# eduard-permyakov/permafrost-engine

Measured on AMD Instinct MI355X. Metric: agent-steps/sec (+ flow-field cells/sec), every chunk field rebuilt + every agent stepped per tick, higher is better.
Workload: dtype u64-bitmask/u8 fields, f32 agents (f64 exp); 1 GPU; BASELINE configs[2]: 1024x1024 cells, 64 flow fields = 16384 chunk fields, 100000 agents; map_chunks=16, flow_fields=64, agents=100000, hz=20, dynamic_obstacles=0, parallelism=requests by destination + uid slabs x1, 1 all-gather (16 B/agent) per tick, ranks=1, rccl_ranks=1, backend=none, tile_exchange=auto, requests=reference planner fixture, has_dest_los=device lookup, initial_velocities=flow aligned, fields_ahead=True, tick_driver=c (navhip_tick_run), library=libnavhip.so (in-tree)

## Files before the change

### permafrost-engine_amd/csrc/field_kernels.hip

```cpp
#include "navhip_internal.h"

#include "wave_bits.h"

__device__ __forceinline__ bool req_uses_bfs(const nh_map_view &map, const navhip_field_req &rq,
                                             int force_generic)
{
    if(force_generic) return false;
    if(rq.type == NAVHIP_TARGET_NEAREST_PATHABLE || (rq.flags & NAVHIP_REQ_ISLAND_NEAREST)) return false;
    const nh_layer_view &L = map.layers[rq.layer];
    return L.unit_cost[(int)rq.chunk_r * map.w + rq.chunk_c] != 0;
}

__device__ __forceinline__ uint16_t portal_first_iid(const uint16_t *li, int r0, int c0, int r1, int c1)
{
    for(int r = r0; r <= r1; r++)
        for(int c = c0; c <= c1; c++) {
            const uint16_t v = li[r * 64 + c];
            if(v != NAVHIP_ISLAND_NONE) return v;
        }
    return NAVHIP_ISLAND_NONE;
}

__device__ __forceinline__ bool req_prepare(const nh_map_view &map, navhip_field_req &rq)
{
    const nh_layer_view &L = map.layers[rq.layer];
    const bool portal = rq.type == NAVHIP_TARGET_PORTAL;
    if((rq.flags & NAVHIP_REQ_IF_CHANGED) && L.changed) {
        bool ch = L.changed[(int)rq.chunk_r * map.w + rq.chunk_c] != 0;
        if(portal) ch |= L.changed[(int)rq.next_chunk_r * map.w + rq.next_chunk_c] != 0;
        if(!ch) return false;
    }
    if((rq.flags & NAVHIP_REQ_LIVE_IIDS) && portal && L.local_islands) {
        rq.port_iid = portal_first_iid(L.local_islands + ((size_t)((int)rq.chunk_r * map.w + rq.chunk_c) << 12),
                                       rq.port_r0, rq.port_c0, rq.port_r1, rq.port_c1);
        rq.next_iid = portal_first_iid(L.local_islands + ((size_t)((int)rq.next_chunk_r * map.w + rq.next_chunk_c) << 12),
                                       rq.next_r0, rq.next_c0, rq.next_r1, rq.next_c1);
        if(rq.port_iid == NAVHIP_ISLAND_NONE || rq.next_iid == NAVHIP_ISLAND_NONE) return false;
    }
    return true;
}

__device__ __forceinline__ bool next_tile_matches(const nh_map_view &map, const navhip_field_req &rq,
                                                  int gr, int gc)
{
    if(gr < 0 || gc < 0) return false;
    int cr2 = gr >> 6, cc2 = gc >> 6, r2 = gr & 63, c2 = gc & 63;
    if(cr2 != rq.next_chunk_r || cc2 != rq.next_chunk_c) return false;
    if(cr2 >= map.h || cc2 >= map.w) return false;
    if(r2 < rq.next_r0 || r2 > rq.next_r1 || c2 < rq.next_c0 || c2 > rq.next_c1) return false;
    const uint16_t *li = map.layers[rq.layer].local_islands;
    return li[((size_t)(cr2 * map.w + cc2) << 12) + r2 * 64 + c2] == rq.next_iid;
}

__device__ __forceinline__ bool portal_seed(const nh_map_view &map, const navhip_field_req &rq,
                                            int r, int c, bool passable)
{
    if(!passable) return false;
    if(r < rq.port_r0 || r > rq.port_r1 || c < rq.port_c0 || c > rq.port_c1) return false;
    const uint16_t *li = map.layers[rq.layer].local_islands;
    size_t cbase = (size_t)((int)rq.chunk_r * map.w + rq.chunk_c) << 12;
    if(rq.port_iid != NAVHIP_ISLAND_NONE && li[cbase + r * 64 + c] != rq.port_iid) return false;
    int gr = rq.chunk_r * 64 + r, gc = rq.chunk_c * 64 + c;
    return next_tile_matches(map, rq, gr - 1, gc) || next_tile_matches(map, rq, gr + 1, gc)
        || next_tile_matches(map, rq, gr, gc - 1) || next_tile_matches(map, rq, gr, gc + 1);
}

__device__ __forceinline__ uint32_t portal_fix_dir(const navhip_field_req &rq)
{
    if(rq.next_chunk_r < rq.chunk_r) return NAVHIP_FD_N;
    if(rq.next_chunk_r > rq.chunk_r) return NAVHIP_FD_S;
    if(rq.next_chunk_c < rq.chunk_c) return NAVHIP_FD_W;
    return NAVHIP_FD_E;
}

__global__ __launch_bounds__(256) void k_derive(const uint8_t *cost, const uint16_t *blockers,
                                                uint64_t *passmask, uint64_t *probemask, uint8_t *unit_cost,
                                                const uint8_t *factions, uint64_t *facmask, uint16_t *facany,
                                                const uint32_t *chunk_list, int n)
{
    int wave = (blockIdx.x * 256 + threadIdx.x) >> 6;
    int lane = threadIdx.x & 63;
    if(wave >= n) return;
    uint32_t chunk = chunk_list ? chunk_list[wave] : (uint32_t)wave;
    const uint8_t  *cb = cost + ((size_t)chunk << 12);
    const uint16_t *bl = blockers ? blockers + ((size_t)chunk << 12) : nullptr;
    uint64_t mine = 0, path = 0, blocked = 0;
    bool nonunit = false;
    for(int r = 0; r < 64; r++) {
        uint32_t cst = cb[r * 64 + lane];
        uint32_t blk = bl ? bl[r * 64 + lane] : 0;
        uint64_t m = __ballot(cst != NAVHIP_COST_IMPASSABLE && blk == 0);
        uint64_t mp = __ballot(cst != NAVHIP_COST_IMPASSABLE), mb = __ballot(blk > 0);
        nonunit |= (cst != NAVHIP_COST_IMPASSABLE && cst != 1);
        if(lane == r) { mine = m; path = mp; blocked = mb; }
    }
    passmask[(size_t)chunk * 64 + lane] = mine;
    probemask[((size_t)chunk * 64 + lane) * 2]     = path;
    probemask[((size_t)chunk * 64 + lane) * 2 + 1] = blocked;
    bool any_nonunit = __any(nonunit);
    if(lane == 0) unit_cost[chunk] = any_nonunit ? 0 : 1;
    if(factions) {
        const uint8_t *fa = factions + ((size_t)chunk * NAVHIP_MAX_FACTIONS << 12) + lane * 64;
        uint32_t any = 0;
        for(int f = 0; f < NAVHIP_MAX_FACTIONS; f++) {
            const uint64_t m = nz_row_mask(fa + ((size_t)f << 12));
            facmask[((size_t)chunk * NAVHIP_MAX_FACTIONS + f) * 64 + lane] = m;
            if(__ballot(m != 0)) any |= 1u << f;
        }
        if(lane == 0) facany[chunk] = (uint16_t)any;
    }
}

void nh_launch_derive(navhip_ctx *ctx, int layer, const uint32_t *d_chunk_list, int n, hipStream_t s)
{
    navhip_layer &L = ctx->layers[layer];
    int blocks = (n + 3) / 4;
    hipLaunchKernelGGL(k_derive, dim3(blocks), dim3(256), 0, s, L.cost, L.blockers, L.passmask, L.probemask,
                       L.unit_cost, L.factions, L.facmask, L.facany, d_chunk_list, n);
}

__device__ __forceinline__ uint64_t faction_pass_row(const nh_layer_view &L, int chunk, int lane, uint32_t enemies)
{
    const uint64_t *pm = L.probemask + ((size_t)chunk * 64 + lane) * 2;
    const uint64_t path = pm[0], blocked = pm[1];
    if(!L.facmask) return path;
    uint64_t friends = 0;
    uint32_t fs = __builtin_amdgcn_readfirstlane((int)(L.facany[chunk] & ~enemies & ((1u << NAVHIP_MAX_FACTIONS) - 1u)));
    const uint64_t *fm = L.facmask + (size_t)chunk * NAVHIP_MAX_FACTIONS * 64 + lane;
    while(fs) {
        const int f = __builtin_ctz(fs);
        fs &= fs - 1;
        friends |= fm[f * 64];
    }
    return path & ~(blocked & friends);
}

#define NH_MAXP 12
#define BFS_WAVES 4

template <bool WANT_INTEG>
__global__ __launch_bounds__(BFS_WAVES * 64) void k_field_bfs(nh_map_view map, const navhip_field_req *reqs,
                                                   int n, uint8_t *dirs, float *integ,
                                                   int force_generic, int32_t *gen_list, int gen_slot,
                                                   const int32_t *out_slot)
{
    __shared__ __attribute__((aligned(16))) uint8_t stage[BFS_WAVES][NH_CELLS];

    const int wib  = threadIdx.x >> 6;
    const int wave = blockIdx.x * BFS_WAVES + wib;
    const int lane = threadIdx.x & 63;
    if(wave >= n) return;

    navhip_field_req rq = reqs[wave];
    if(!req_uses_bfs(map, rq, force_generic)) {
        if(lane == 0) gen_list[2 + atomicAdd(&gen_list[gen_slot], 1)] = wave;
        return;
    }
    if(!req_prepare(map, rq)) return;

    const nh_layer_view &L = map.layers[rq.layer];
    const int chunk = (int)rq.chunk_r * map.w + rq.chunk_c;
    const u64x pass = mk(rq.faction_id == NAVHIP_FACTION_ID_NONE ? L.passmask[(size_t)chunk * 64 + lane]
                                                                 : faction_pass_row(L, chunk, lane, rq.enemies));

    u64x seeds = u64x{0, 0};
    if(rq.type == NAVHIP_TARGET_TILE) {
        if(lane == rq.tile_r) seeds = mk(1ull << rq.tile_c) & pass;
    }else{
        if(rq.port_c0 == rq.port_c1) {
            bool s = portal_seed(map, rq, lane, rq.port_c0, (to64(pass) >> rq.port_c0) & 1);
            if(s) seeds = mk(1ull << rq.port_c0);
        }else{
            for(int r = rq.port_r0; r <= rq.port_r1; r++) {
                uint64_t prow = __shfl(to64(pass), r);
                bool s = portal_seed(map, rq, r, lane, (prow >> lane) & 1);
                uint64_t m = __ballot(s);
                if(lane == r) seeds = mk(m);
            }
        }
    }

    u64x open = andn(pass, seeds);
    u64x frontier = seeds;
    u64x pl[NH_MAXP];
#pragma unroll
    for(int k = 0; k < NH_MAXP; k++) pl[k] = u64x{0, 0};

    int level = 0;
#define NH_BFS_LEVEL(NLOW)                                                                   \
    {                                                                                        \
        u64x nw = bfs_reach(frontier, open);                                                 \
        if(!__any(nz(nw))) break;                                                            \
        level++;                                                                             \
        pl[0] = pl[0] ^ open;                                                                \
        if(NLOW > 1) pl[1] = pl[1] ^ open;                                                   \
        if(NLOW > 2) pl[2] = pl[2] ^ open;                                                   \
        if(NLOW > 3) {                                                                       \
            const int tz = __builtin_ctz(level);          \
            _Pragma("unroll")                                                                \
            for(int k = 3; k < NH_MAXP; k++) {                                               \
                if(k <= tz) pl[k] = pl[k] ^ open;                                            \
            }                                                                                \
        }                                                                                    \
        open = andn(open, nw);                                                               \
        frontier = nw;                                                                       \
    }
    for(;;) {
        NH_BFS_LEVEL(1) NH_BFS_LEVEL(2) NH_BFS_LEVEL(1) NH_BFS_LEVEL(3)
        NH_BFS_LEVEL(1) NH_BFS_LEVEL(2) NH_BFS_LEVEL(1) NH_BFS_LEVEL(4)
    }
#undef NH_BFS_LEVEL
    const u64x reach = andn(pass, open);
#pragma unroll
    for(int k = 0; k < NH_MAXP; k++) pl[k] = pl[k] & reach;

    const int P = 32 - __builtin_clz((unsigned)level + 1);

    if(WANT_INTEG) {
        float *out = integ + ((size_t)wave << 12);
        for(int c = 0; c < 64; c++) {
            uint32_t d = 0;
#pragma unroll
            for(int k = 0; k < NH_MAXP; k++) d |= (uint32_t)((to64(pl[k]) >> c) & 1) << k;
            bool fin = (to64(reach) >> c) & 1;
            out[lane * 64 + c] = fin ? (float)d : __builtin_inff();
        }
    }

    u64x anybit = u64x{0, 0};
#pragma unroll
    for(int k = 0; k < NH_MAXP; k++) anybit = anybit | pl[k];
    const u64x zero = andn(reach, anybit);
    const u64x act  = reach & anybit;

    const u64x rN = from_n(reach), rS = from_s(reach), rW = from_w(reach), rE = from_e(reach);
    u64x eqN, eqS, eqW, eqE;
    {
        const u64x m0 = pl[0], m1 = pl[1];
        u64x n0, n1;
        n0 = from_n(pl[0]); n1 = from_n(pl[1]); eqN = andn(n0 ^ m0, n1 ^ n0 ^ m1) & rN;
        n0 = from_s(pl[0]); n1 = from_s(pl[1]); eqS = andn(n0 ^ m0, n1 ^ n0 ^ m1) & rS;
        n0 = from_w(pl[0]); n1 = from_w(pl[1]); eqW = andn(n0 ^ m0, n1 ^ n0 ^ m1) & rW;
        n0 = from_e(pl[0]); n1 = from_e(pl[1]); eqE = andn(n0 ^ m0, n1 ^ n0 ^ m1) & rE;
    }

    u64x neNW = u64x{0, 0}, neNE = neNW, neSW = neNW, neSE = neNW;
    {
        u64x b1 = u64x{~0u, ~0u};
        u64x b2 = u64x{~0u, ~0u};
#pragma unroll
        for(int k = 0; k < NH_MAXP; k++) {
            if(k < P) {
                u64x e = pl[k] ^ b1;  b1 = andn(b1, pl[k]);
                u64x f = e ^ b2;      b2 = andn(b2, e);
                u64x up = from_n(pl[k]), dn = from_s(pl[k]);
                neNW = neNW | (from_w(up) ^ f);
                neNE = neNE | (from_e(up) ^ f);
                neSW = neSW | (from_w(dn) ^ f);
                neSE = neSE | (from_e(dn) ^ f);
            }
        }
    }
    const u64x eqNW = andn(from_w(rN), neNW), eqNE = andn(from_e(rN), neNE);
    const u64x eqSW = andn(from_w(rS), neSW), eqSE = andn(from_e(rS), neSE);

    const u64x hasD = (eqNW & rN & rW) | (eqNE & rN & rE) | (eqSW & rS & rW) | (eqSE & rS & rE);
    const u64x h = act & hasD;
    const u64x g = andn(act, hasD);

    const u64x mN  = g & eqN;
    const u64x mS  = andn(g & eqS, eqN);
    const u64x mE  = andn(g & eqE, eqN | eqS);
    const u64x mW  = andn(g & eqW, eqN | eqS | eqE);
    const u64x mNW = h & eqNW;
    const u64x mNE = andn(h & eqNE, eqNW);
    const u64x mSW = andn(h & eqSW, eqNW | eqNE);
    const u64x mSE = andn(h & eqSE, eqNW | eqNE | eqSW);

    u64x D0 = mNW | mNE | mE | mS;
    u64x D1 = mN | mNE | mSW | mS;
    u64x D2 = mW | mE | mSW | mS;
    u64x D3 = mSE;
    if(rq.type == NAVHIP_TARGET_PORTAL) {
        uint32_t fd = portal_fix_dir(rq);
        if(fd & 1) D0 = D0 | zero;
        if(fd & 2) D1 = D1 | zero;
        if(fd & 4) D2 = D2 | zero;
    }

    uint8_t *out = dirs + ((size_t)(out_slot ? out_slot[wave] : wave) << 12);
    uint8_t *st = stage[wib];
    const bool inout = (rq.flags & NAVHIP_REQ_INOUT) != 0;
    if(inout) {
#pragma unroll
        for(int j = 0; j < 4; j++)
            *(uint4*)(st + j * 1024 + lane * 16) = *(const uint4*)(out + j * 1024 + lane * 16);
    }
    __builtin_amdgcn_wave_barrier();
    {
        uint32_t *row = (uint32_t*)(st + lane * 64);
        const uint64_t d0 = to64(D0), d1 = to64(D1), d2 = to64(D2), d3 = to64(D3);
        const uint64_t rc = to64(reach);
#pragma unroll
        for(int j = 0; j < 16; j++) {
            uint32_t b0 = (((uint32_t)(d0 >> (4 * j)) & 0xf) * 0x00204081u) & 0x01010101u;
            uint32_t b1 = (((uint32_t)(d1 >> (4 * j)) & 0xf) * 0x00204081u) & 0x01010101u;
            uint32_t b2 = (((uint32_t)(d2 >> (4 * j)) & 0xf) * 0x00204081u) & 0x01010101u;
            uint32_t b3 = (((uint32_t)(d3 >> (4 * j)) & 0xf) * 0x00204081u) & 0x01010101u;
            uint32_t v = b0 | (b1 << 1) | (b2 << 2) | (b3 << 3);
            if(inout) {
                uint32_t rm = ((((uint32_t)(rc >> (4 * j)) & 0xf) * 0x00204081u) & 0x01010101u) * 0xffu;
                v = (v & rm) | (row[j] & ~rm);
            }
            row[j] = v;
        }
    }
    __builtin_amdgcn_wave_barrier();
#pragma unroll
    for(int j = 0; j < 4; j++)
        *(uint4*)(out + j * 1024 + lane * 16) = *(const uint4*)(st + j * 1024 + lane * 16);
}

struct generic_lds {
    uint32_t dist[NH_CELLS];
    __attribute__((aligned(16))) uint8_t pc[NH_CELLS];
    uint8_t raw[NH_CELLS];
    uint8_t fl[NH_CELLS];
    int s_list[128], s_dmin[128], s_nlist, s_D;
};

__device__ void field_generic_one(generic_lds &S, const nh_map_view &map, const navhip_field_req *reqs,
                                  int ri, uint8_t *dirs, float *integ, int force_generic,
                                  const int32_t *out_slot)
{
    uint32_t (&dist)[NH_CELLS] = S.dist;
    uint8_t (&pc)[NH_CELLS] = S.pc;
    uint8_t (&raw)[NH_CELLS] = S.raw;
    uint8_t (&fl)[NH_CELLS] = S.fl;
    int (&s_list)[128] = S.s_list;
    int (&s_dmin)[128] = S.s_dmin;
    int &s_nlist = S.s_nlist, &s_D = S.s_D;

    const int t = threadIdx.x;
    navhip_field_req rq = reqs[ri];
    if(req_uses_bfs(map, rq, force_generic)) return;
    if(!req_prepare(map, rq)) return;

    const nh_layer_view &L = map.layers[rq.layer];
    const size_t cbase = (size_t)((int)rq.chunk_r * map.w + rq.chunk_c) << 12;
    const bool faction = rq.faction_id != NAVHIP_FACTION_ID_NONE;
    const bool modeA = rq.type == NAVHIP_TARGET_NEAREST_PATHABLE;
    const bool modeB = !modeA && (rq.flags & NAVHIP_REQ_ISLAND_NEAREST) != 0;

#pragma unroll 4
    for(int k = 0; k < 16; k++) {
        int i = k * 256 + t;
        uint32_t cst = L.cost[cbase + i];
        uint32_t blk = L.blockers ? L.blockers[cbase + i] : 0;
        bool passable;
        if(cst == NAVHIP_COST_IMPASSABLE) {
            passable = false;
        }else if(!faction) {
            passable = (blk == 0);
        }else{
            bool enemies_only = true;
            if(L.factions) {
                const uint8_t *fp = L.factions + cbase * NAVHIP_MAX_FACTIONS + i;
                for(int f = 0; f < NAVHIP_MAX_FACTIONS; f++) {
                    if(fp[(size_t)f << 12] && !(rq.enemies & (1u << f))) { enemies_only = false; break; }
                }
            }
            passable = enemies_only || (blk == 0);
        }
        pc[i] = passable ? (uint8_t)cst : (uint8_t)NAVHIP_COST_IMPASSABLE;
        raw[i] = (uint8_t)cst;
        fl[i] = (cst != NAVHIP_COST_IMPASSABLE && blk == 0) ? 1 : 0;
        dist[i] = NH_INF_U32;
    }
    if(t == 0) { s_nlist = 0; s_D = 0x7fffffff; }
    if(t < 128) s_dmin[t] = 0x7fffffff;
    __syncthreads();

    if(modeA) {
        const int start = rq.tile_r * 64 + rq.tile_c;
        if(t == 0) fl[start] |= 2;
        __syncthreads();
        if(!(fl[start] & 1)) {
            for(;;) {
                int changed = 0;
#pragma unroll 4
                for(int k = 0; k < 16; k++) {
                    int i = k * 256 + t;
                    if(fl[i] & 3) continue;
                    int r = i >> 6, c = i & 63;
                    bool nb = (r > 0 && (fl[i - 64] & 2)) || (r < 63 && (fl[i + 64] & 2))
                           || (c > 0 && (fl[i - 1] & 2)) || (c < 63 && (fl[i + 1] & 2));
                    if(nb) { fl[i] |= 2; changed = 1; }
                }
                if(!__syncthreads_or(changed)) break;
            }
#pragma unroll 4
            for(int k = 0; k < 16; k++) {
                int i = k * 256 + t;
                if(!(fl[i] & 1)) continue;
                int r = i >> 6, c = i & 63;
                bool nb = (r > 0 && (fl[i - 64] & 2)) || (r < 63 && (fl[i + 64] & 2))
                       || (c > 0 && (fl[i - 1] & 2)) || (c < 63 && (fl[i + 1] & 2));
                if(nb) dist[i] = 0;
            }
        }else if(t == 0) {
            dist[start] = 0;
        }
        __syncthreads();
        for(;;) {
            int changed = 0;
#pragma unroll 4
            for(int k = 0; k < 16; k++) {
                int i = k * 256 + t;
                if(fl[i] & 1) continue;
                int r = i >> 6, c = i & 63;
                uint32_t m = NH_INF_U32;
                if(r > 0)  m = min(m, dist[i - 64]);
                if(r < 63) m = min(m, dist[i + 64]);
                if(c > 0)  m = min(m, dist[i - 1]);
                if(c < 63) m = min(m, dist[i + 1]);
                if(m < NH_INF_U32) {
                    uint32_t nd = m + raw[i];
                    if(nd < dist[i]) { dist[i] = nd; changed = 1; }
                }
            }
            if(!__syncthreads_or(changed)) break;
        }
    }else{
        if(rq.type == NAVHIP_TARGET_TILE) {
            if(t == 0) {
                int i = rq.tile_r * 64 + rq.tile_c;
                if(pc[i] != NAVHIP_COST_IMPASSABLE) {
                    if(modeB) s_list[s_nlist++] = i; else dist[i] = 0;
                }
            }
        }else{
            int nr = rq.port_r1 - rq.port_r0 + 1, nc = rq.port_c1 - rq.port_c0 + 1;
            for(int j = t; j < nr * nc; j += 256) {
                int r = rq.port_r0 + j / nc, c = rq.port_c0 + j % nc;
                if(portal_seed(map, rq, r, c, pc[r * 64 + c] != NAVHIP_COST_IMPASSABLE)) {
                    if(modeB) { int p = atomicAdd(&s_nlist, 1); if(p < 128) s_list[p] = r * 64 + c; }
                    else dist[r * 64 + c] = 0;
                }
            }
        }
        __syncthreads();
        if(modeB) {
            if(t == 0 && s_nlist == 0 && rq.type == NAVHIP_TARGET_TILE)
                s_list[s_nlist++] = rq.tile_r * 64 + rq.tile_c;
            __syncthreads();
            const int nl = min(s_nlist, 128);
            const uint16_t *li = L.local_islands + cbase;
            const uint16_t *gi = L.islands ? L.islands + cbase : nullptr;
            const uint32_t want = rq.aux_iid;
            for(int q = 0; q < nl; q++) {
                const int f = s_list[q], fr = f >> 6, fc = f & 63;
                const uint32_t giid = gi ? gi[f] : NAVHIP_ISLAND_NONE;
                int best = 0x7fffffff;
#pragma unroll 4
                for(int k = 0; k < 16; k++) {
                    int i = k * 256 + t;
                    if(!(fl[i] & 1)) continue;
                    if(want != NAVHIP_ISLAND_NONE && li[i] != want) continue;
                    if(giid != NAVHIP_ISLAND_NONE && gi[i] != giid) continue;
                    int d = abs((i >> 6) - fr) + abs((i & 63) - fc);
                    best = min(best, d);
                }
                if(best < 0x7fffffff) atomicMin(&s_dmin[q], best);
            }
            __syncthreads();
            if(t == 0) {
                int D = 0x7fffffff;
                for(int q = 0; q < nl; q++) D = min(D, s_dmin[q]);
                s_D = D;
            }
            __syncthreads();
            const int D = s_D;
            if(D < 0x7fffffff) {
                for(int q = 0; q < nl; q++) {
                    if(s_dmin[q] != D) continue;
                    const int f = s_list[q], fr = f >> 6, fc = f & 63;
                    const uint32_t giid = gi ? gi[f] : NAVHIP_ISLAND_NONE;
#pragma unroll 4
                    for(int k = 0; k < 16; k++) {
                        int i = k * 256 + t;
                        if(!(fl[i] & 1)) continue;
                        if(want != NAVHIP_ISLAND_NONE && li[i] != want) continue;
                        if(giid != NAVHIP_ISLAND_NONE && gi[i] != giid) continue;
                        if(abs((i >> 6) - fr) + abs((i & 63) - fc) == D) dist[i] = 0;
                    }
                }
            }
            __syncthreads();
        }

        for(;;) {
            int changed = 0;
#pragma unroll 4
            for(int k = 0; k < 16; k++) {
                int i = k * 256 + t;
                uint32_t cst = pc[i];
                if(cst == NAVHIP_COST_IMPASSABLE) continue;
                int r = i >> 6, c = i & 63;
                uint32_t m = NH_INF_U32;
                if(r > 0)  m = min(m, dist[i - 64]);
                if(r < 63) m = min(m, dist[i + 64]);
                if(c > 0)  m = min(m, dist[i - 1]);
                if(c < 63) m = min(m, dist[i + 1]);
                if(m < NH_INF_U32) {
                    uint32_t nd = m + cst;
                    if(nd < dist[i]) { dist[i] = nd; changed = 1; }
                }
            }
            if(!__syncthreads_or(changed)) break;
        }
    }

    const bool inout = (rq.flags & NAVHIP_REQ_INOUT) != 0 || modeA || modeB;
    uint8_t *out = dirs + ((size_t)(out_slot ? out_slot[ri] : ri) << 12);
    const uint32_t fixdir = (rq.type == NAVHIP_TARGET_PORTAL) ? portal_fix_dir(rq) : NAVHIP_FD_NONE;
    uint8_t res[16];
#pragma unroll 4
    for(int k = 0; k < 16; k++) {
        int i = k * 256 + t;
        int r = i >> 6, c = i & 63;
        uint32_t d = dist[i];
        uint32_t dir;
        if(d >= NH_INF_U32) {
            dir = inout ? out[i] : NAVHIP_FD_NONE;
        }else if(d == 0) {
            dir = modeA ? out[i] : fixdir;
        }else{
            const uint32_t I = NH_INF_U32;
            uint32_t dn = r > 0  ? dist[i - 64] : I, ds = r < 63 ? dist[i + 64] : I;
            uint32_t dw = c > 0  ? dist[i - 1]  : I, de = c < 63 ? dist[i + 1]  : I;
            uint32_t dnw = (r > 0  && c > 0)  ? dist[i - 65] : I;
            uint32_t dne = (r > 0  && c < 63) ? dist[i - 63] : I;
            uint32_t dsw = (r < 63 && c > 0)  ? dist[i + 63] : I;
            uint32_t dse = (r < 63 && c < 63) ? dist[i + 65] : I;
            uint32_t mc = min(min(dn, ds), min(dw, de));
            if(dn < I && dw < I) mc = min(mc, dnw);
            if(dn < I && de < I) mc = min(mc, dne);
            if(ds < I && dw < I) mc = min(mc, dsw);
            if(ds < I && de < I) mc = min(mc, dse);
            if(dn == mc)       dir = NAVHIP_FD_N;
            else if(ds == mc)  dir = NAVHIP_FD_S;
            else if(de == mc)  dir = NAVHIP_FD_E;
            else if(dw == mc)  dir = NAVHIP_FD_W;
            else if(dnw == mc) dir = NAVHIP_FD_NW;
            else if(dne == mc) dir = NAVHIP_FD_NE;
            else if(dsw == mc) dir = NAVHIP_FD_SW;
            else               dir = NAVHIP_FD_SE;
        }
        res[k] = (uint8_t)dir;
        if(integ) integ[((size_t)ri << 12) + i] = (d >= NH_INF_U32) ? __builtin_inff() : (float)d;
    }
    __syncthreads();
#pragma unroll
    for(int k = 0; k < 16; k++) pc[k * 256 + t] = res[k];
    __syncthreads();
    *(uint4*)(out + t * 16) = *(const uint4*)(pc + t * 16);
}

__global__ __launch_bounds__(256) void k_field_generic(nh_map_view map, const navhip_field_req *reqs,
                                                       int n, uint8_t *dirs, float *integ,
                                                       int force_generic, int32_t *gen_list, int gen_slot,
                                                       const int32_t *out_slot)
{
    __shared__ generic_lds S;
    const int count = gen_list ? gen_list[gen_slot] : n;
    if(gen_list && blockIdx.x == 0 && threadIdx.x == 0) gen_list[gen_slot ^ 1] = 0;
    for(int w = blockIdx.x; w < count; w += gridDim.x) {
        const int ri = gen_list ? gen_list[2 + w] : w;
        field_generic_one(S, map, reqs, ri, dirs, integ, force_generic, out_slot);
        __syncthreads();
    }
}

int nh_launch_fields(navhip_ctx *ctx, const navhip_field_req *d_reqs, int n, uint8_t *d_dirs,
                     float *d_integ, int32_t *d_gen_list, hipStream_t s, const int32_t *d_out_slot)
{
    nh_map_view mv;
    nh_fill_map_view(ctx, &mv);
    const int force_generic = ctx->field_kernel_mode == 1;
    const int gen_slot = force_generic ? 0 : (int)(ctx->gen_launches++ & 1);
    if(!force_generic) {
        dim3 grid((n + BFS_WAVES - 1) / BFS_WAVES);
        if(d_integ)
            hipLaunchKernelGGL(k_field_bfs<true>, grid, dim3(BFS_WAVES * 64), 0, s, mv, d_reqs, n, d_dirs,
                               d_integ, force_generic, d_gen_list, gen_slot, d_out_slot);
        else
            hipLaunchKernelGGL(k_field_bfs<false>, grid, dim3(BFS_WAVES * 64), 0, s, mv, d_reqs, n, d_dirs,
                               d_integ, force_generic, d_gen_list, gen_slot, d_out_slot);
    }
    bool heavy = force_generic;
    for(int l = 0; l < NAVHIP_NAV_LAYER_MAX; l++) heavy = heavy || (ctx->layers[l].cost && ctx->layers[l].nonunit_costs);
    const int gmax = heavy ? 2048 : 512;
    hipLaunchKernelGGL(k_field_generic, dim3(n < gmax ? n : gmax), dim3(256), 0, s, mv, d_reqs, n, d_dirs,
                       d_integ, force_generic, force_generic ? (int32_t*)nullptr : d_gen_list, gen_slot, d_out_slot);
    return force_generic ? -1 : gen_slot;
}
```

Baseline: 39.02 million agent-steps/s.

## Skip high distance-plane diagonal comparisons unless detour cells exist in BFS field kernel

Makes the BFS level counter and wave index wave-uniform with readfirstlane and turns the higher-plane XOR updates into an early-break loop. It drops the per-plane masking by the reach set. It also reorders the diagonal-equality computation so the planes at index 3 and above are only processed when some active cell has a diagonal neighbour not reachable through its orthogonal neighbours. The borrow chain is seeded from the low planes so the high planes run first. This is meant to cut ALU and register pressure in the flow-field build, at the cost of a subtle correctness argument that the low planes alone decide diagonal equality when there are no detours.

Result: no change. 39.41 million agent-steps/s, median of 6 (+1.0%).

```diff
diff --git a/permafrost-engine_amd/csrc/field_kernels.hip b/permafrost-engine_amd/csrc/field_kernels.hip
--- a/permafrost-engine_amd/csrc/field_kernels.hip
+++ b/permafrost-engine_amd/csrc/field_kernels.hip
@@ -146,7 +146,7 @@
 {
     __shared__ __attribute__((aligned(16))) uint8_t stage[BFS_WAVES][NH_CELLS];
 
-    const int wib  = threadIdx.x >> 6;
+    const int wib  = __builtin_amdgcn_readfirstlane(threadIdx.x >> 6);
     const int wave = blockIdx.x * BFS_WAVES + wib;
     const int lane = threadIdx.x & 63;
     if(wave >= n) return;
@@ -196,10 +196,12 @@
         if(NLOW > 1) pl[1] = pl[1] ^ open;                                                   \
         if(NLOW > 2) pl[2] = pl[2] ^ open;                                                   \
         if(NLOW > 3) {                                                                       \
-            const int tz = __builtin_ctz(level);          \
+            const int tz = __builtin_amdgcn_readfirstlane(__builtin_ctz(level));             \
+            pl[3] = pl[3] ^ open;                                                            \
             _Pragma("unroll")                                                                \
-            for(int k = 3; k < NH_MAXP; k++) {                                               \
-                if(k <= tz) pl[k] = pl[k] ^ open;                                            \
+            for(int k = 4; k < NH_MAXP; k++) {                                               \
+                if(k > tz) break;                                                            \
+                pl[k] = u64x{nh_keep32(pl[k].lo ^ open.lo), nh_keep32(pl[k].hi ^ open.hi)};  \
             }                                                                                \
         }                                                                                    \
         open = andn(open, nw);                                                               \
@@ -211,8 +213,6 @@
     }
 #undef NH_BFS_LEVEL
     const u64x reach = andn(pass, open);
-#pragma unroll
-    for(int k = 0; k < NH_MAXP; k++) pl[k] = pl[k] & reach;
 
     const int P = 32 - __builtin_clz((unsigned)level + 1);
 
@@ -234,6 +234,38 @@
     const u64x act  = reach & anybit;
 
     const u64x rN = from_n(reach), rS = from_s(reach), rW = from_w(reach), rE = from_e(reach);
+
+    const u64x dNW = from_w(rN), dNE = from_e(rN), dSW = from_w(rS), dSE = from_e(rS);
+    const u64x detour = act & (andn(dNW, rN | rW) | andn(dNE, rN | rE) | andn(dSW, rS | rW) | andn(dSE, rS | rE));
+    const bool high_planes = P > 3 && __any(nz(detour));
+    u64x neNW = u64x{0, 0}, neNE = neNW, neSW = neNW, neSE = neNW;
+    {
+        u64x b1, b2;
+#define NH_DIAG_PLANE(k)                                                                     \
+        {                                                                                    \
+            u64x e = pl[k] ^ b1;  b1 = andn(b1, pl[k]);                                      \
+            u64x f = e ^ b2;      b2 = andn(b2, e);                                          \
+            u64x up = from_n(pl[k]), dn = from_s(pl[k]);                                     \
+            neNW = neNW | (from_w(up) ^ f);                                                  \
+            neNE = neNE | (from_e(up) ^ f);                                                  \
+            neSW = neSW | (from_w(dn) ^ f);                                                  \
+            neSE = neSE | (from_e(dn) ^ f);                                                  \
+        }
+        if(high_planes) {
+            b1 = andn(~pl[0], pl[1] | pl[2]);
+            b2 = andn(pl[0], pl[1] | pl[2]);
+#pragma unroll
+            for(int k = 3; k < NH_MAXP; k++) {
+                if(k < P) NH_DIAG_PLANE(k)
+            }
+        }
+        b1 = b2 = u64x{~0u, ~0u};
+        NH_DIAG_PLANE(0) NH_DIAG_PLANE(1) NH_DIAG_PLANE(2)
+#undef NH_DIAG_PLANE
+    }
+    const u64x eqNW = andn(dNW, neNW), eqNE = andn(dNE, neNE);
+    const u64x eqSW = andn(dSW, neSW), eqSE = andn(dSE, neSE);
+
     u64x eqN, eqS, eqW, eqE;
     {
         const u64x m0 = pl[0], m1 = pl[1];
@@ -243,26 +275,6 @@
         n0 = from_w(pl[0]); n1 = from_w(pl[1]); eqW = andn(n0 ^ m0, n1 ^ n0 ^ m1) & rW;
         n0 = from_e(pl[0]); n1 = from_e(pl[1]); eqE = andn(n0 ^ m0, n1 ^ n0 ^ m1) & rE;
     }
-
-    u64x neNW = u64x{0, 0}, neNE = neNW, neSW = neNW, neSE = neNW;
-    {
-        u64x b1 = u64x{~0u, ~0u};
-        u64x b2 = u64x{~0u, ~0u};
-#pragma unroll
-        for(int k = 0; k < NH_MAXP; k++) {
-            if(k < P) {
-                u64x e = pl[k] ^ b1;  b1 = andn(b1, pl[k]);
-                u64x f = e ^ b2;      b2 = andn(b2, e);
-                u64x up = from_n(pl[k]), dn = from_s(pl[k]);
-                neNW = neNW | (from_w(up) ^ f);
-                neNE = neNE | (from_e(up) ^ f);
-                neSW = neSW | (from_w(dn) ^ f);
-                neSE = neSE | (from_e(dn) ^ f);
-            }
-        }
-    }
-    const u64x eqNW = andn(from_w(rN), neNW), eqNE = andn(from_e(rN), neNE);
-    const u64x eqSW = andn(from_w(rS), neSW), eqSE = andn(from_e(rS), neSE);
 
     const u64x hasD = (eqNW & rN & rW) | (eqNE & rN & rE) | (eqSW & rS & rW) | (eqSE & rS & rE);
     const u64x h = act & hasD;
```
